# spacejam/loghisto

Hardware: NVIDIA H100
Metric: histogram ingest throughput (samples/s) (higher is better)
Workload: dtype f64

## Files before the change

loghisto_b200/csrc/lh_api.cu:

```cuda
#include "../../include/loghisto_b200.h"
#include "lh_kernels.cuh"

#include <algorithm>
#include <cmath>
#include <condition_variable>
#include <cstdio>
#include <cstring>
#include <mutex>
#include <new>
#include <string>
#include <thread>
#include <vector>
#include <unistd.h>

using namespace lh;

namespace {

struct WriterEvent { cudaStream_t stream; cudaEvent_t ev; };

struct Scope { uint64_t ticket; int buf; cudaStream_t stream; std::thread::id thread; };
static_assert(sizeof(Prec) == sizeof(((lh_recorder *)0)->prec) && offsetof(lh_recorder, prec) % alignof(Prec) == 0,
              "lh_recorder.prec must hold an lh::Prec");

// ... 154 lines not shown
    int nnz_slot = 0;
    short *d_x_keys = nullptr; unsigned long long *d_x_counts = nullptr; size_t x_cap = 0;
    uint32_t *h_offsets = nullptr;
    short *h_x_keys = nullptr; unsigned long long *h_x_counts = nullptr; size_t hx_cap = 0;
    unsigned long long *h_counter_deltas = nullptr;
    std::vector<Slot> slots;
    uint64_t slot_seq = 0;
    size_t staging_bytes = 0;
    unsigned long long last_margin[2] = {0, 0};
    int k1_variant = kDefaultK1Variant;
    int k1_grid_mult = 1;
    int k1_reserve_sms = 0;
    int keyed_blocks_per_sm = 8;
    uint32_t hot_replicas = 1;
    int keyed_mode = 0;
    int64_t kp_chunk = 256 << 20;
    uint32_t wc_pf_tiles = 1;
    uint32_t wc_flush_samples = 24576;
    int wc_spt = 6;
    unsigned short *d_kp_queues = nullptr;
    unsigned int *d_kp_cnt = nullptr;
    uint4 *d_kp_rare = nullptr;
    size_t kp_cap = 0;
    int kp_parts = 0;
    const char *keyed_kernel = "";
    int batch_blocks_per_sm = 1;
    BatchParams batch_prm{};
    uint32_t comm_rank = 0, comm_world = 0;
    unsigned long long *d_comm = nullptr;
    unsigned int *d_comm_aux = nullptr;
    PeerMap peers[kMaxRanks];
    unsigned long long *d_red_buckets = nullptr;
    uint32_t *d_red_flags = nullptr;
    unsigned long long *d_red_counters = nullptr;
// ... 177 lines not shown

template <typename IdT, typename ValT>
void launch_keyed_scalar(lh_ctx *ctx, const KeyedOut &ko, const IdT *ids, const ValT *vals, size_t n, cudaStream_t s,
                         const IdMap *map = nullptr) {
    if (!n) return;
    constexpr int T = 256;
    const int grid = grid_1d(ctx, n, T, 1, ctx->keyed_blocks_per_sm);
    if (map) k_ingest_keyed<IdT, ValT, T, IdMap><<<grid, T, (size_t)map->k * 4, s>>>(ids, vals, n, ko, ctx->pc, *map);
    else k_ingest_keyed<IdT, ValT, T><<<grid, T, 0, s>>>(ids, vals, n, ko, ctx->pc, IdIdentity{});
    ctx->stats.kernel_launches++;
}

constexpr uint32_t KS_MAX_PASSES = 4;

constexpr size_t kSmemBudget = 227 * 1024;

struct KeyedPlan {
    enum Route { SCALAR , SMALL, WC, VEC, APART } route = SCALAR;
    const char *name = "k_ingest_keyed";
    size_t head = 0, n4 = 0;
    size_t taken = 0, taken2 = 0;
    int grid = 0;
    size_t smem = 0;
    uint32_t per = 0;
    int spt = 0, threads = 0;
    WcParams wc{};
};

KeyedPlan plan_keyed(const lh_ctx *ctx, uint32_t nids, size_t id_bytes, const void *ids, const void *vals, size_t n, bool pair = false,
                     const void *ids2 = nullptr, const void *vals2 = nullptr, size_t n2 = 0) {
    KeyedPlan p;
    if (!nids) return p;
    const uint32_t ks_per_max = std::max<uint32_t>(1, (uint32_t)(KS_SMEM_BYTES / ((size_t)ctx->pc.win * 4)));
    const uint32_t ks_passes = (nids + ks_per_max - 1) / ks_per_max;
    const bool small = ks_passes <= KS_MAX_PASSES && ctx->keyed_mode == 0;
    const uintptr_t id_mask = 4 * id_bytes - 1;
    if (pair) {
        auto aligned = [&](const void *v, const void *i) { return ((uintptr_t)v & 31u) == 0 && ((uintptr_t)i & id_mask) == 0; };
        p.route = KeyedPlan::APART;
        if (!n || !n2 || ctx->keyed_mode == 1 || small || !aligned(vals, ids) || !aligned(vals2, ids2)) return p;
// ... 6 lines not shown
        if (small && p.n4 >= 4096) {
            p.route = KeyedPlan::SMALL; p.name = "k_ingest_keyed_small";
            p.per = (nids + ks_passes - 1) / ks_passes;
            p.smem = ((size_t)p.per * ctx->pc.win + 4) * 4;
            p.grid = (int)std::max<size_t>(1, std::min<size_t>((size_t)(ctx->sm_count - ctx->k1_reserve_sms),
                                                               p.n4 / (KS_THREADS * 16)));
            return p;
        }
        p.route = KeyedPlan::VEC; p.name = "k_ingest_keyed_vec";
        if (ctx->keyed_mode == 1) return p;
    }
    const int P = std::min(ctx->sm_count - ctx->k1_reserve_sms, (int)WC_MAX_PARTS);
    if (P < 8) return p;
    const uint32_t ids_per = (nids + P - 1) / P;
    const size_t hist_bytes = (((size_t)ids_per * ctx->pc.win + 3) & ~(size_t)3) * 4;
    uint32_t row_cap = 0;
    size_t smem = 0;
    for (uint32_t cap_try : {256u, 192u, 128u}) {
        smem = hist_bytes + 2 * WC_MAX_PARTS * 4 + (size_t)(P + 1) * (cap_try + WC_ROW_EXTRA) * 2;
        if (smem <= kSmemBudget) { row_cap = cap_try; break; }
    }
    if (!row_cap || (size_t)ids_per * ctx->pc.win > 65535) return p;
    if (ctx->keyed_mode != 2 && n + n2 < ((size_t)1 << 22)) return p;
    const int spt = ctx->wc_spt == 6 || ctx->wc_spt == 4 || ctx->wc_spt == 3 ? ctx->wc_spt : 8;
    const int tile = spt == 6 ? WcShape<6>::TILE : spt == 4 ? WcShape<4>::TILE : spt == 3 ? WcShape<3>::TILE : WcShape<8>::TILE;
    const size_t taken = n / tile * tile, taken2 = n2 / tile * tile;
    if (taken + taken2 == 0) return p;
    p.route = KeyedPlan::WC; p.name = "k_ingest_keyed_wc";
    p.taken = taken; p.taken2 = taken2; p.grid = P; p.smem = smem; p.spt = spt;
    p.threads = spt == 6 ? WcShape<6>::THREADS : spt == 4 ? WcShape<4>::THREADS : spt == 3 ? WcShape<3>::THREADS : WcShape<8>::THREADS;
    WcParams &w = p.wc;
    w.n = taken; w.n2 = taken2; w.ids_per = ids_per; w.row_cap = row_cap; w.row_stride = row_cap + WC_ROW_EXTRA;
    w.inv_p = (uint32_t)(((uint64_t)1 << 32) / (uint64_t)P) + 1u;
    w.pf_tiles = ctx->wc_pf_tiles;
    const size_t slice_max = std::max<size_t>(1, ((size_t)ctx->kp_chunk + (size_t)P * tile - 1) / ((size_t)P * tile));
    const size_t tiles_all = taken / tile + taken2 / tile;
    const size_t nchunks = (tiles_all + slice_max * P - 1) / (slice_max * P);
    w.slice_tiles = (uint32_t)std::max<size_t>(1, (tiles_all + nchunks * P - 1) / (nchunks * P));
    const size_t expect = slice_max * tile / P;
    w.cap = (uint32_t)(((expect * 5 / 4 + 3 * WC_LINE + WC_LINE - 1) / WC_LINE) * WC_LINE);
    const double room = (double)row_cap - 63.0;
    const double m_max = std::pow((-3.5 + std::sqrt(3.5 * 3.5 + 4.0 * room)) / 2.0, 2.0);
    const uint32_t flush_samples = std::min<uint32_t>(ctx->wc_flush_samples, (uint32_t)(m_max * P));
    w.flush_tiles = std::max<uint32_t>(1u, flush_samples / tile);
    return p;
}

std::mutex g_wc_mu;
std::vector<cudaEvent_t> g_wc_done;

cudaError_t wc_done_event(int device, cudaEvent_t *out) {
    if ((size_t)device >= g_wc_done.size()) g_wc_done.resize((size_t)device + 1, nullptr);
    if (!g_wc_done[device]) {
        cudaError_t e = cudaEventCreateWithFlags(&g_wc_done[device], cudaEventDisableTiming);
        if (e != cudaSuccess) { g_wc_done[device] = nullptr; return e; }
    }
    *out = g_wc_done[device];
    return cudaSuccess;
}

template <typename IdT, typename ValT>
lh_status launch_keyed_wc(lh_ctx *ctx, int b, const KeyedPlan &p, const IdT *ids, const ValT *vals, cudaStream_t s,
                          const IdT *ids2 = nullptr, const long long *vals2 = nullptr, const IdMap *map = nullptr) {
    const int P = p.grid;
    if (!ctx->d_kp_queues || ctx->kp_cap != p.wc.cap || ctx->kp_parts != P) {
        if (ctx->d_kp_queues) {
            cudaEvent_t done;
            {
                std::lock_guard<std::mutex> lk(g_wc_mu);
                LH_CUDA(ctx, wc_done_event(ctx->device, &done));
            }
            LH_CUDA(ctx, cudaEventSynchronize(done));
        }
        cudaFree(ctx->d_kp_queues); cudaFree(ctx->d_kp_cnt); cudaFree(ctx->d_kp_rare);
        ctx->d_kp_queues = nullptr; ctx->d_kp_cnt = nullptr; ctx->d_kp_rare = nullptr;
        LH_CUDA(ctx, cudaMalloc(&ctx->d_kp_rare, (size_t)P * WC_RARE_CAP * sizeof(uint4)));
        LH_CUDA(ctx, cudaMalloc(&ctx->d_kp_queues, (size_t)2 * P * P * p.wc.cap * sizeof(unsigned short)));
        LH_CUDA(ctx, cudaMalloc(&ctx->d_kp_cnt, ((size_t)2 * P * P + 1) * sizeof(unsigned int)));
        ctx->kp_cap = p.wc.cap; ctx->kp_parts = P;
    }
#define LH_WC_KERNEL(SPT) (!p.taken2 ? (const void *)k_ingest_keyed_wc<IdT, ValT, SPT, false> : (const void *)k_ingest_keyed_wc<IdT, double, SPT, true>)
    const void *fn = p.spt == 6 ? LH_WC_KERNEL(6) : p.spt == 4 ? LH_WC_KERNEL(4) : p.spt == 3 ? LH_WC_KERNEL(3) : LH_WC_KERNEL(8);
#undef LH_WC_KERNEL
#define LH_WC_MAPPED(SPT) (const void *)k_ingest_keyed_wc<IdT, ValT, SPT, false, IdMap>
    if (map) fn = p.spt == 6 ? LH_WC_MAPPED(6) : p.spt == 4 ? LH_WC_MAPPED(4) : p.spt == 3 ? LH_WC_MAPPED(3) : LH_WC_MAPPED(8);
#undef LH_WC_MAPPED
    LH_CUDA(ctx, cudaFuncSetAttribute(fn, cudaFuncAttributeMaxDynamicSharedMemorySize, (int)kSmemBudget));
    WcParams prm = p.wc;
    prm.ids = ids; prm.vals = vals; prm.ids2 = ids2; prm.vals2 = vals2;
    prm.queues = ctx->d_kp_queues; prm.q_cnt = ctx->d_kp_cnt; prm.barrier = ctx->d_kp_cnt + (size_t)2 * P * P;
    prm.rare = ctx->d_kp_rare; prm.o = keyed_out(ctx, b);
    Prec pc = ctx->pc;
    IdIdentity ident;
    void *args[] = {&prm, &pc, map ? (void *)map : (void *)&ident};
    {
        std::lock_guard<std::mutex> lk(g_wc_mu);
        cudaEvent_t done;
        LH_CUDA(ctx, wc_done_event(ctx->device, &done));
        LH_CUDA(ctx, cudaStreamWaitEvent(s, done, 0));
        LH_CUDA(ctx, cudaMemsetAsync(prm.barrier, 0, sizeof(unsigned int), s));
        LH_CUDA(ctx, cudaLaunchCooperativeKernel(fn, dim3(P), dim3(p.threads), args, p.smem, s));
        LH_CUDA(ctx, cudaEventRecord(done, s));
    }
    ctx->stats.kernel_launches++;
    return LH_OK;
}

template <typename IdT, typename ValT>
lh_status launch_keyed(lh_ctx *ctx, int b, const IdT *d_ids, const ValT *d_vals, size_t n, cudaStream_t s,
                       const IdMap *map = nullptr) {
    constexpr int T = 256;
    const uint32_t nids = map ? map->k : ctx->H;
    const KeyedOut ko = keyed_out(ctx, b);
    size_t done = 0;
    while (done < n) {
        const unsigned long long kCap = 0xFFFFFFFFull;
        if (ctx->buf[b].hot_pending >= kCap - (1ull << 30)) {
            for (const WriterEvent &w : ctx->buf[b].writers)
                if (w.stream != s) LH_CUDA(ctx, cudaStreamWaitEvent(s, w.ev, 0));
// ... 2325 lines not shown
        ctx->keyed_mode = (int)value;
        return LH_OK;
    }
    if (!strcmp(key, "wc_pf")) {
        if (value < 0 || value > 8) return fail(ctx, LH_ERR_RANGE, "wc_pf is 0 ... 8 tiles");
        ctx->wc_pf_tiles = (uint32_t)value;
        return LH_OK;
    }
    if (!strcmp(key, "wc_flush")) {
        if (value < 4096 || value > 65536) return fail(ctx, LH_ERR_RANGE, "wc_flush is 4096 ... 65536 samples");
        ctx->wc_flush_samples = (uint32_t)value;
        return LH_OK;
    }
    if (!strcmp(key, "wc_spt")) {
        if (value != 4 && value != 6 && value != 3 && value != 8)
            return fail(ctx, LH_ERR_RANGE, "wc_spt is a shape code: 6 (896 threads x 4 samples), 4 (1024 x 4), 3 (768 x 4) or 8 (512 x 8)");
        ctx->wc_spt = (int)value;
        return LH_OK;
    }
    if (!strcmp(key, "kp_chunk")) {
        if (value < (1 << 16) || value > ((int64_t)1 << 28)) return fail(ctx, LH_ERR_RANGE, "kp_chunk out of range");
        ctx->kp_chunk = value;
        return LH_OK;
    }
    if (!strcmp(key, "gpu_timer_slots")) {
        if (value < 1 || value > (1 << 20)) return fail(ctx, LH_ERR_RANGE, "gpu_timer_slots is 1 ... 2^20");
        if (ctx->d_timer_marks) return fail(ctx, LH_ERR_STATE, "gpu_timer_slots is set before the first lh_gpu_timer_start");
        ctx->timer_slots_n = (uint32_t)value;
        return LH_OK;
    }
    if (!strcmp(key, "keyed_blocks_per_sm")) {
        if (value < 1 || value > 32) return fail(ctx, LH_ERR_RANGE, "keyed_blocks_per_sm out of range");
        ctx->keyed_blocks_per_sm = (int)value;
        return LH_OK;
    }
    return fail(ctx, LH_ERR_INVALID, "unknown tuning key");
// ... 35 lines not shown
```

loghisto_b200/csrc/lh_kernels.cuh:

```cuda
#pragma once
#include "../../include/loghisto_b200.h"
#include <type_traits>
#include "lh_device.cuh"

namespace lh {

struct f64x4 { double a, b, c, d; };
__device__ __forceinline__ uint64_t policy_evict_first() {
    uint64_t p;
    asm("createpolicy.fractional.L2::evict_first.b64 %0, 1.0;" : "=l"(p));
    return p;
}
__device__ __forceinline__ void ldg_stream_u64x4(const void *p, unsigned long long (&r)[4]) {
    const uint64_t pol = policy_evict_first();
    asm volatile("ld.global.nc.L1::no_allocate.L2::cache_hint.v2.b64 {%0, %1}, [%2], %3;"
                 : "=l"(r[0]), "=l"(r[1]) : "l"(p), "l"(pol));
    asm volatile("ld.global.nc.L1::no_allocate.L2::cache_hint.v2.b64 {%0, %1}, [%2], %3;"
                 : "=l"(r[2]), "=l"(r[3]) : "l"((const char *)p + 16), "l"(pol));
}
__device__ __forceinline__ f64x4 ldg_stream_f64x4(const void *p) {
    unsigned long long u[4];
    ldg_stream_u64x4(p, u);
    f64x4 r;
    r.a = __longlong_as_double((long long)u[0]); r.b = __longlong_as_double((long long)u[1]);
// ... 496 lines not shown
        const uint32_t c = ks_hist[i];
        if (!c) continue;
        const uint32_t lid = i / row, slot = i - lid * row;
        const uint32_t r = mv.row(id_lo + lid);
        if (kMapped<Map> && r == 0xFFFFFFFFu) atomicAdd(o.dropped, (unsigned long long)c);
        else atomicAdd(&o.hot[(size_t)r * (2u * pc.win) + slot], c);
    }
}

constexpr int WC_MAX_PARTS = 160;
constexpr int WC_LINE = 64;

template <int SPT> struct WcShape {
    static constexpr int THREADS = SPT == 4 ? 1024 : SPT == 6 ? 896 : SPT == 3 ? 768 : 512;
    static constexpr int PER = SPT == 8 ? 8 : 4;
    static constexpr int TILE = THREADS * PER;
};
constexpr int WC_ROW_EXTRA = WC_LINE + 8;

struct WcParams {
    const void *ids;
    const void *vals;
    size_t n;
    const void *ids2;
    const void *vals2;
    size_t n2;
    uint32_t ids_per;
    uint32_t cap;
    uint32_t slice_tiles;
    uint32_t inv_p;
    uint32_t flush_tiles;
    uint32_t pf_tiles;
    uint32_t row_cap;
    uint32_t row_stride;
    unsigned short *queues;
    unsigned int *q_cnt;
    unsigned int *barrier;
    uint4 *rare;
    KeyedOut o;
};
constexpr uint32_t WC_RARE_CAP = 8192;

__device__ __forceinline__ void grid_barrier(unsigned int *bar, unsigned int target) {
    __syncthreads();
    if (threadIdx.x == 0) {
        __threadfence();
        atomicAdd(bar, 1u);
        unsigned int v;
        do {
            asm volatile("ld.acquire.gpu.global.u32 %0, [%1];" : "=r"(v) : "l"(bar) : "memory");
        } while (v < target);
    }
    __syncthreads();
}

template <typename V = IdIdentity>
__device__ __forceinline__ void wc_spill(uint32_t rec, uint32_t owner, uint32_t P, const Prec &pc, const KeyedOut &o, const V &m = {}) {
    const uint32_t lid = rec / pc.win, slot = rec - lid * pc.win, id = m.row(lid * P + owner);
    if (kMapped<V> && id == 0xFFFFFFFFu) { atomicAdd(o.dropped, 1ull); return; }
    add_bucket_global(o.buckets + (size_t)id * 65536u, o.flags + id, slot, 1ull, pc.win);
}

template <typename IdT, typename ValT, int SPT, bool PAIR = false, typename Map = IdIdentity>
__global__ void __launch_bounds__(WcShape<SPT>::THREADS, 1)
k_ingest_keyed_wc(WcParams prm, Prec pc, const Map map) {
    static_assert(!PAIR || std::is_same<ValT, double>::value, "the int64 segment rides on the float64 instantiation");
    static_assert(!PAIR || !kMapped<Map>, "pairs are not mapped");
    const auto mv = map_view(map);
    using S = WcShape<SPT>;
    constexpr int WC_THREADS = S::THREADS;
    constexpr int GROUPS = S::PER / 4;
    extern __shared__ __align__(16) unsigned char wc_smem[];
    const uint32_t P = gridDim.x, p = blockIdx.x, tid = threadIdx.x;
    unsigned int *s_hist = reinterpret_cast<unsigned int *>(wc_smem);
    const uint32_t hist_words = prm.ids_per * pc.win;
    unsigned int *s_fill = s_hist + ((hist_words + 3u) & ~3u);
    unsigned int *s_off = s_fill + WC_MAX_PARTS;
    unsigned short *s_buf = reinterpret_cast<unsigned short *>(s_off + WC_MAX_PARTS);
    uint32_t fill_addr = smem_u32(s_fill);
    const uint32_t hist_addr = smem_u32(s_hist);
    asm volatile("mov.b32 %0, %0;" : "+r"(fill_addr));
    const uint32_t buf_addr = fill_addr + 2u * WC_MAX_PARTS * 4u;
    unsigned int *s_rare = s_fill + (WC_MAX_PARTS - 1);
    uint4 *rareq = prm.rare + (size_t)p * WC_RARE_CAP;
    uint32_t negP = 0u - P;
    asm volatile("mov.b32 %0, %0;" : "+r"(negP));

    for (uint32_t i = tid; i < hist_words; i += WC_THREADS) s_hist[i] = 0;
    if (tid < WC_MAX_PARTS) { s_fill[tid] = 0; s_off[tid] = 0; }
    uint32_t one_bits;
    asm volatile("mov.b32 %0, 0x3F800000;" : "=r"(one_bits));
    __syncthreads();

    const size_t tiles_seg0 = prm.n / S::TILE;
    const size_t tiles_total = tiles_seg0 + (PAIR ? prm.n2 / S::TILE : 0);
    const size_t chunk_tiles = (size_t)prm.slice_tiles * P;
    const size_t nchunks = (tiles_total + chunk_tiles - 1) / chunk_tiles;
    const IdT *ids = reinterpret_cast<const IdT *>(prm.ids);
    const unsigned int cap = prm.cap;
    const uint32_t row_cap = prm.row_cap, row_stride = prm.row_stride;


    unsigned long long cur[GROUPS][4], nxt[GROUPS][4];
    IdPack<IdT> cur_id[GROUPS], nxt_id[GROUPS];
    uint32_t since_flush = 0;
    const char *vptr = nullptr;
    const IdT *iptr = nullptr;
    const size_t pf_v = (size_t)prm.pf_tiles * S::TILE * 8, pf_i = (size_t)prm.pf_tiles * S::TILE;
    auto load_tile = [&](const char *vp, const IdT *ip, unsigned long long (&raw)[GROUPS][4], IdPack<IdT> (&idp)[GROUPS]) {
#pragma unroll
        for (int g = 0; g < GROUPS; g++) {
            load_vals4(vp, (size_t)g * WC_THREADS, raw[g]);
            idp[g].load(ip, (size_t)g * WC_THREADS);
        }
    };

    for (size_t c = 0; c < nchunks; c++) {
        const size_t par = c & 1;
        unsigned short *qset = prm.queues + par * (size_t)P * P * cap;
        unsigned int *cset = prm.q_cnt + par * (size_t)P * P;
        const bool last_chunk = c + 1 == nchunks;
        const size_t tile0 = c * chunk_tiles + (size_t)p * prm.slice_tiles;
        const uint32_t ntile_all = tile0 >= tiles_total ? 0u : (uint32_t)min((size_t)prm.slice_tiles, tiles_total - tile0);
        auto bin_tile = [&](unsigned long long (&raw)[GROUPS][4], IdPack<IdT> (&idp)[GROUPS], const bool as_i64) {
            if constexpr (PAIR) {
                if (as_i64) {
#pragma unroll
                    for (int g = 0; g < GROUPS; g++)
#pragma unroll
                        for (int j = 0; j < 4; j++) raw[g][j] = (unsigned long long)__double_as_longlong(__ll2double_rn((long long)raw[g][j]));
                }
            }
#pragma unroll
            for (int g = 0; g < GROUPS; g++) {
                double v[4];
#pragma unroll
                for (int j = 0; j < 4; j++) { ValT r; memcpy(&r, &raw[g][j], 8); v[j] = sample_to_f64<ValT>(r); }
                uint32_t idx[4];
                bool flag[4];
                bucket_offsets_v2<4, false, 0>(v, pc, one_bits, idx, flag);
                bool any = false;
#pragma unroll
                for (int j = 0; j < 4; j++) {
                    const uint32_t id = idp[g].get(j);
                    const uint32_t lid = __umulhi(id, prm.inv_p), owner = lid * negP + id;
                    const uint32_t rec = lid * pc.win + idx[j];
                    const bool rare = flag[j] | (id >= mv.bound(prm.o.H));
                    const uint32_t oe = rare ? P : owner;
                    uint32_t pos;
                    asm volatile("atom.shared.add.u32 %0, [%1], 1;" : "=r"(pos) : "r"(fill_addr + oe * 4u) : "memory");
                    flag[j] = rare | (pos >= row_cap);
                    if (!flag[j])
                        asm volatile("st.shared.u16 [%0], %1;" ::"r"(buf_addr + (oe * row_stride + pos) * 2u), "h"((unsigned short)rec) : "memory");
                    any |= flag[j];
                }
                if (__any_sync(0xFFFFFFFFu, any)) {
#pragma unroll
                    for (int j = 0; j < 4; j++)
                        if (flag[j]) {
                            const unsigned int at = atomicAdd(s_rare, 1u);
                            if (at < WC_RARE_CAP) rareq[at] = make_uint4((unsigned int)raw[g][j], (unsigned int)(raw[g][j] >> 32), idp[g].get(j), 0u);
                            else keyed_one_slow_v<ValT>(idp[g].get(j), raw[g][j], pc, prm.o, mv);
                        }
                }
            }
            if (++since_flush == prm.flush_tiles) {
                since_flush = 0;
                __syncthreads();
                constexpr uint32_t GROUPS_PER_WARP = 8;
                const uint32_t sub = (tid & 31) >> 2, k4 = (tid & 3) * 2;
                for (uint32_t base = (tid >> 5) * GROUPS_PER_WARP; base < P; base += (WC_THREADS / 32) * GROUPS_PER_WARP) {
                    const uint32_t o = base + sub;
                    const bool act = o < P;
                    unsigned int n = 0, nfull = 0, off0 = 0;
                    uint4 keep0 = make_uint4(0, 0, 0, 0), keep1 = keep0;
                    uint4 *src = reinterpret_cast<uint4 *>(s_buf + (act ? o : 0) * row_stride);
                    if (act) {
                        n = min(s_fill[o], row_cap);
                        nfull = n / WC_LINE;
                        off0 = s_off[o];
                        unsigned short *qbase = qset + ((size_t)o * P + p) * cap;
                        keep0 = src[nfull * 8 + k4];
                        keep1 = src[nfull * 8 + k4 + 1];
                        for (unsigned int l = 0; l < nfull; l++) {
                            if (off0 + WC_LINE <= cap) {
                                uint4 *dst = reinterpret_cast<uint4 *>(qbase + off0);
                                const uint4 a0 = src[l * 8 + k4], a1 = src[l * 8 + k4 + 1];
                                dst[k4] = a0;
                                dst[k4 + 1] = a1;
                                off0 += WC_LINE;
                            } else if (k4 == 0) {
                                const unsigned short *r = s_buf + o * row_stride + l * WC_LINE;
                                for (unsigned int k = 0; k < (unsigned int)WC_LINE; k++) wc_spill(r[k], o, P, pc, prm.o, mv);
                            }
                        }
                    }
                    __syncwarp();
                    if (act) {
                        if (nfull) { src[k4] = keep0; src[k4 + 1] = keep1; }
                        if (k4 == 0) { s_off[o] = off0; s_fill[o] = n - nfull * WC_LINE; }
                    }
                }
                __syncthreads();
            }
        };
        for (int part = 0; part < (PAIR ? 2 : 1); part++) {
            const size_t lo = part == 0 ? tile0 : max(tile0, tiles_seg0);
            const size_t hi = part == 0 ? min(tile0 + ntile_all, tiles_seg0) : tile0 + ntile_all;
            if (hi <= lo) continue;
            const uint32_t ntile = (uint32_t)(hi - lo);
            const bool as_i64 = part == 1;
            const size_t first = (part == 0 ? lo : lo - tiles_seg0) * S::TILE + (size_t)tid * 4;
            vptr = reinterpret_cast<const char *>(part == 0 ? prm.vals : prm.vals2) + first * 8;
            iptr = (part == 0 ? ids : reinterpret_cast<const IdT *>(prm.ids2)) + first;
            load_tile(vptr, iptr, cur, cur_id);
            auto prefetch_ahead = [&](uint32_t tile_loaded) {
                if (prm.pf_tiles && tile_loaded + prm.pf_tiles < ntile) {
#pragma unroll
                    for (int g = 0; g < GROUPS; g++) {
                        asm volatile("prefetch.global.L2 [%0];" ::"l"(vptr + pf_v + (size_t)g * WC_THREADS * 32));
                        if ((tid & 3) == 0) asm volatile("prefetch.global.L2 [%0];" ::"l"(iptr + pf_i + (size_t)g * WC_THREADS * 4));
                    }
                }
            };
            for (uint32_t t = 0; t < ntile; t += 2) {
                vptr += (size_t)S::TILE * 8;
                iptr += S::TILE;
                if (t + 1 < ntile) load_tile(vptr, iptr, nxt, nxt_id);
                prefetch_ahead(t + 1);
                bin_tile(cur, cur_id, as_i64);
                if (t + 1 >= ntile) break;
                vptr += (size_t)S::TILE * 8;
                iptr += S::TILE;
                if (t + 2 < ntile) load_tile(vptr, iptr, cur, cur_id);
                prefetch_ahead(t + 2);
                bin_tile(nxt, nxt_id, as_i64);
            }
        }
        __syncthreads();
        {
            const unsigned int nr = min(*s_rare, WC_RARE_CAP);
            for (unsigned int i = tid; i < nr; i += WC_THREADS) {
                const uint4 e = rareq[i];
                ValT r;
                const unsigned long long raw = ((unsigned long long)e.y << 32) | e.x;
                memcpy(&r, &raw, 8);
                keyed_one_direct<ValT>(e.z, r, pc, prm.o, mv);
            }
            __syncthreads();
            if (tid == 0) *s_rare = 0;
        }
        if (last_chunk) {
            if (tid < P) {
                const uint32_t o = tid;
                const unsigned int n = min(s_fill[o], row_cap);
                unsigned int off0 = s_off[o];
                const uint4 *src = reinterpret_cast<const uint4 *>(s_buf + o * row_stride);
                for (unsigned int l = 0; l * WC_LINE < n; l++) {
                    const unsigned int nrec = min((unsigned int)WC_LINE, n - l * WC_LINE);
                    if (off0 + WC_LINE <= cap) {
                        uint4 *dst = reinterpret_cast<uint4 *>(qset + ((size_t)o * P + p) * cap + off0);
#pragma unroll
                        for (int k = 0; k < 8; k++) dst[k] = src[l * 8 + k];
                        off0 += nrec;
                    } else {
                        const unsigned short *r = s_buf + o * row_stride + l * WC_LINE;
                        for (unsigned int k = 0; k < nrec; k++) wc_spill(r[k], o, P, pc, prm.o, mv);
                    }
                }
                s_off[o] = off0;
                s_fill[o] = 0;
            }
            __syncthreads();
        }
        if (tid < P) { cset[(size_t)tid * P + p] = s_off[tid]; }
        grid_barrier(prm.barrier, (unsigned int)((c + 1) * (size_t)P));
        if (tid < P) s_off[tid] = __ldcg(&cset[(size_t)p * P + tid]);
        __syncthreads();
        {
            const unsigned short *qmine = qset + (size_t)p * P * cap;
            const uint32_t lane = tid & 31;
#define LH_WC_INC2(word)                                                                                              \
            asm volatile("red.shared.add.u32 [%0], 1;" ::"r"(hist_addr + (((word) << 2) & 0x3FFFCu)) : "memory");     \
            asm volatile("red.shared.add.u32 [%0], 1;" ::"r"(hist_addr + (((word) >> 14) & 0x3FFFCu)) : "memory");
            for (uint32_t w = tid >> 5; w < P; w += WC_THREADS / 32) {
                const unsigned int cnt = s_off[w];
                const unsigned short *q = qmine + (size_t)w * cap;
                const uint4 *qv = reinterpret_cast<const uint4 *>(q);
                const unsigned int nv = cnt >> 3;
#pragma unroll 2
                for (unsigned int i = lane; i < nv; i += 32) {
                    const uint4 v4 = __ldcg(qv + i);
                    LH_WC_INC2(v4.x) LH_WC_INC2(v4.y) LH_WC_INC2(v4.z) LH_WC_INC2(v4.w)
                }
                const unsigned int r0 = nv * 8u + lane;
                if (r0 < cnt) asm volatile("red.shared.add.u32 [%0], 1;" ::"r"(hist_addr + (unsigned int)__ldcg(q + r0) * 4u) : "memory");
            }
#undef LH_WC_INC2
        }
        __syncthreads();
        if (tid < P) s_off[tid] = 0;
    }
    __syncthreads();
    for (uint32_t lid = 0; lid < prm.ids_per; lid++) {
        if (lid * P + p >= mv.bound(prm.o.H)) break;
        const uint32_t id = mv.row(lid * P + p);
        if (kMapped<Map> && id == 0xFFFFFFFFu) {
            unsigned long long lost = 0;
            for (uint32_t slot = tid; slot < pc.win; slot += WC_THREADS) lost += s_hist[lid * pc.win + slot];
            if (lost) atomicAdd(prm.o.dropped, lost);
            continue;
        }
        int any = 0;
        for (uint32_t slot = tid; slot < pc.win; slot += WC_THREADS) {
            const unsigned int cnt = s_hist[lid * pc.win + slot];
            if (cnt) { atomicAdd(&prm.o.buckets[(size_t)id * 65536u + slot], (unsigned long long)cnt); any = 1; }
        }
        any = __syncthreads_or(any);
        if (any && tid == 0) mark(&prm.o.flags[id], 1u);
    }
}

__global__ void k_fold_hot(unsigned int *__restrict__ hot, unsigned long long *__restrict__ buckets, uint32_t *__restrict__ flags,
                           size_t cells, uint32_t replicas, uint32_t win) {
    const size_t stride = (size_t)gridDim.x * blockDim.x;
    const uint32_t row = 2u * win;
    for (size_t i = (size_t)blockIdx.x * blockDim.x + threadIdx.x; i < cells; i += stride) {
        unsigned long long sum = 0;
        for (uint32_t r = 0; r < replicas; r++) {
// ... 1587 lines not shown
```

Measured before the change: 399.4 billion.

## Split cooperative keyed write-combine kernel into per-chunk bin and drain launches

Replaces the single cooperative kernel, which used software grid barriers and double-buffered queues, with two ordinary kernels per chunk. The first bins samples using twice as many writer CTAs, two per SM, each with a smaller shared budget. The second drains the queues into per-owner shared histograms. This removes the grid-barrier spin and the large per-CTA shared footprint in exchange for extra launches, re-zeroing and flushing the histograms on every chunk, and losing overlap between binning and draining. Defaults also change to a larger chunk and the 3-sample shape.

```diff
diff --git a/loghisto_b200/csrc/lh_api.cu b/loghisto_b200/csrc/lh_api.cu
--- a/loghisto_b200/csrc/lh_api.cu
+++ b/loghisto_b200/csrc/lh_api.cu
@@ -192,10 +192,10 @@
     int keyed_blocks_per_sm = 8;
     uint32_t hot_replicas = 1;
     int keyed_mode = 0;
-    int64_t kp_chunk = 256 << 20;
+    int64_t kp_chunk = 512 << 20;
     uint32_t wc_pf_tiles = 1;
     uint32_t wc_flush_samples = 24576;
-    int wc_spt = 6;
+    int wc_spt = 3;
     unsigned short *d_kp_queues = nullptr;
     unsigned int *d_kp_cnt = nullptr;
     uint4 *d_kp_rare = nullptr;
@@ -403,6 +403,8 @@
 constexpr uint32_t KS_MAX_PASSES = 4;
 
 constexpr size_t kSmemBudget = 227 * 1024;
+constexpr size_t kBinSmemBudget = 113 * 1024;
+constexpr size_t kWcQueueBytes = (size_t)5 << 28;
 
 struct KeyedPlan {
     enum Route { SCALAR , SMALL, WC, VEC, APART } route = SCALAR;
@@ -413,6 +415,8 @@
     size_t smem = 0;
     uint32_t per = 0;
     int spt = 0, threads = 0;
+    size_t drain_smem = 0;
+    uint32_t nchunks = 0;
     WcParams wc{};
 };
 
@@ -449,29 +453,31 @@
     if (P < 8) return p;
     const uint32_t ids_per = (nids + P - 1) / P;
     const size_t hist_bytes = (((size_t)ids_per * ctx->pc.win + 3) & ~(size_t)3) * 4;
-    uint32_t row_cap = 0;
-    size_t smem = 0;
-    for (uint32_t cap_try : {256u, 192u, 128u}) {
-        smem = hist_bytes + 2 * WC_MAX_PARTS * 4 + (size_t)(P + 1) * (cap_try + WC_ROW_EXTRA) * 2;
-        if (smem <= kSmemBudget) { row_cap = cap_try; break; }
-    }
-    if (!row_cap || (size_t)ids_per * ctx->pc.win > 65535) return p;
+    bool reach = false;
+    for (uint32_t cap_try : {256u, 192u, 128u})
+        reach = reach || hist_bytes + 2 * WC_MAX_PARTS * 4 + (size_t)(P + 1) * (cap_try + WC_ROW_EXTRA) * 2 <= kSmemBudget;
+    if (!reach || (size_t)ids_per * ctx->pc.win > 65535) return p;
     if (ctx->keyed_mode != 2 && n + n2 < ((size_t)1 << 22)) return p;
-    const int spt = ctx->wc_spt == 6 || ctx->wc_spt == 4 || ctx->wc_spt == 3 ? ctx->wc_spt : 8;
-    const int tile = spt == 6 ? WcShape<6>::TILE : spt == 4 ? WcShape<4>::TILE : spt == 3 ? WcShape<3>::TILE : WcShape<8>::TILE;
+    const int spt = ctx->wc_spt == 8 ? 8 : 3;
+    const int tile = spt == 3 ? WcShape<3>::TILE : WcShape<8>::TILE;
     const size_t taken = n / tile * tile, taken2 = n2 / tile * tile;
     if (taken + taken2 == 0) return p;
+    const int W = 2 * P;
+    const uint32_t row_cap = (uint32_t)(((kBinSmemBudget - wc_bin_smem(P, 0)) / ((size_t)(P + 1) * 2) - WC_ROW_EXTRA) / WC_LINE * WC_LINE);
     p.route = KeyedPlan::WC; p.name = "k_ingest_keyed_wc";
-    p.taken = taken; p.taken2 = taken2; p.grid = P; p.smem = smem; p.spt = spt;
-    p.threads = spt == 6 ? WcShape<6>::THREADS : spt == 4 ? WcShape<4>::THREADS : spt == 3 ? WcShape<3>::THREADS : WcShape<8>::THREADS;
+    p.taken = taken; p.taken2 = taken2; p.grid = P; p.spt = spt;
+    p.threads = spt == 3 ? WcShape<3>::CTA_THREADS : WcShape<8>::CTA_THREADS;
+    p.smem = wc_bin_smem(P, row_cap + WC_ROW_EXTRA);
+    p.drain_smem = hist_bytes + (size_t)W * 4;
     WcParams &w = p.wc;
-    w.n = taken; w.n2 = taken2; w.ids_per = ids_per; w.row_cap = row_cap; w.row_stride = row_cap + WC_ROW_EXTRA;
+    w.n = taken; w.n2 = taken2; w.parts = P; w.writers = W; w.ids_per = ids_per; w.row_cap = row_cap; w.row_stride = row_cap + WC_ROW_EXTRA;
     w.inv_p = (uint32_t)(((uint64_t)1 << 32) / (uint64_t)P) + 1u;
     w.pf_tiles = ctx->wc_pf_tiles;
-    const size_t slice_max = std::max<size_t>(1, ((size_t)ctx->kp_chunk + (size_t)P * tile - 1) / ((size_t)P * tile));
+    const size_t chunk = std::min<size_t>((size_t)ctx->kp_chunk, kWcQueueBytes * 2 / 5);
+    const size_t slice_max = std::max<size_t>(1, (chunk + (size_t)W * tile - 1) / ((size_t)W * tile));
     const size_t tiles_all = taken / tile + taken2 / tile;
-    const size_t nchunks = (tiles_all + slice_max * P - 1) / (slice_max * P);
-    w.slice_tiles = (uint32_t)std::max<size_t>(1, (tiles_all + nchunks * P - 1) / (nchunks * P));
+    p.nchunks = (uint32_t)((tiles_all + slice_max * W - 1) / (slice_max * W));
+    w.slice_tiles = (uint32_t)std::max<size_t>(1, (tiles_all + (size_t)p.nchunks * W - 1) / ((size_t)p.nchunks * W));
     const size_t expect = slice_max * tile / P;
     w.cap = (uint32_t)(((expect * 5 / 4 + 3 * WC_LINE + WC_LINE - 1) / WC_LINE) * WC_LINE);
     const double room = (double)row_cap - 63.0;
@@ -497,7 +503,7 @@
 template <typename IdT, typename ValT>
 lh_status launch_keyed_wc(lh_ctx *ctx, int b, const KeyedPlan &p, const IdT *ids, const ValT *vals, cudaStream_t s,
                           const IdT *ids2 = nullptr, const long long *vals2 = nullptr, const IdMap *map = nullptr) {
-    const int P = p.grid;
+    const int P = p.grid, W = (int)p.wc.writers;
     if (!ctx->d_kp_queues || ctx->kp_cap != p.wc.cap || ctx->kp_parts != P) {
         if (ctx->d_kp_queues) {
             cudaEvent_t done;
@@ -509,21 +515,21 @@
         }
         cudaFree(ctx->d_kp_queues); cudaFree(ctx->d_kp_cnt); cudaFree(ctx->d_kp_rare);
         ctx->d_kp_queues = nullptr; ctx->d_kp_cnt = nullptr; ctx->d_kp_rare = nullptr;
-        LH_CUDA(ctx, cudaMalloc(&ctx->d_kp_rare, (size_t)P * WC_RARE_CAP * sizeof(uint4)));
-        LH_CUDA(ctx, cudaMalloc(&ctx->d_kp_queues, (size_t)2 * P * P * p.wc.cap * sizeof(unsigned short)));
-        LH_CUDA(ctx, cudaMalloc(&ctx->d_kp_cnt, ((size_t)2 * P * P + 1) * sizeof(unsigned int)));
+        LH_CUDA(ctx, cudaMalloc(&ctx->d_kp_rare, (size_t)W * WC_RARE_CAP * sizeof(uint4)));
+        LH_CUDA(ctx, cudaMalloc(&ctx->d_kp_queues, (size_t)P * W * p.wc.cap * sizeof(unsigned short)));
+        LH_CUDA(ctx, cudaMalloc(&ctx->d_kp_cnt, (size_t)P * W * sizeof(unsigned int)));
         ctx->kp_cap = p.wc.cap; ctx->kp_parts = P;
     }
-#define LH_WC_KERNEL(SPT) (!p.taken2 ? (const void *)k_ingest_keyed_wc<IdT, ValT, SPT, false> : (const void *)k_ingest_keyed_wc<IdT, double, SPT, true>)
-    const void *fn = p.spt == 6 ? LH_WC_KERNEL(6) : p.spt == 4 ? LH_WC_KERNEL(4) : p.spt == 3 ? LH_WC_KERNEL(3) : LH_WC_KERNEL(8);
+#define LH_WC_KERNEL(SPT) (map ? (const void *)k_keyed_bin<IdT, ValT, SPT, false, IdMap> : !p.taken2 ? (const void *)k_keyed_bin<IdT, ValT, SPT, false> \
+                                                                                    : (const void *)k_keyed_bin<IdT, double, SPT, true>)
+    const void *bin = p.spt == 3 ? LH_WC_KERNEL(3) : LH_WC_KERNEL(8);
 #undef LH_WC_KERNEL
-#define LH_WC_MAPPED(SPT) (const void *)k_ingest_keyed_wc<IdT, ValT, SPT, false, IdMap>
-    if (map) fn = p.spt == 6 ? LH_WC_MAPPED(6) : p.spt == 4 ? LH_WC_MAPPED(4) : p.spt == 3 ? LH_WC_MAPPED(3) : LH_WC_MAPPED(8);
-#undef LH_WC_MAPPED
-    LH_CUDA(ctx, cudaFuncSetAttribute(fn, cudaFuncAttributeMaxDynamicSharedMemorySize, (int)kSmemBudget));
+    const void *drain = map ? (const void *)k_keyed_drain<IdMap> : (const void *)k_keyed_drain<IdIdentity>;
+    LH_CUDA(ctx, cudaFuncSetAttribute(bin, cudaFuncAttributeMaxDynamicSharedMemorySize, (int)kBinSmemBudget));
+    LH_CUDA(ctx, cudaFuncSetAttribute(drain, cudaFuncAttributeMaxDynamicSharedMemorySize, (int)kSmemBudget));
     WcParams prm = p.wc;
     prm.ids = ids; prm.vals = vals; prm.ids2 = ids2; prm.vals2 = vals2;
-    prm.queues = ctx->d_kp_queues; prm.q_cnt = ctx->d_kp_cnt; prm.barrier = ctx->d_kp_cnt + (size_t)2 * P * P;
+    prm.queues = ctx->d_kp_queues; prm.q_cnt = ctx->d_kp_cnt;
     prm.rare = ctx->d_kp_rare; prm.o = keyed_out(ctx, b);
     Prec pc = ctx->pc;
     IdIdentity ident;
@@ -533,11 +539,14 @@
         cudaEvent_t done;
         LH_CUDA(ctx, wc_done_event(ctx->device, &done));
         LH_CUDA(ctx, cudaStreamWaitEvent(s, done, 0));
-        LH_CUDA(ctx, cudaMemsetAsync(prm.barrier, 0, sizeof(unsigned int), s));
-        LH_CUDA(ctx, cudaLaunchCooperativeKernel(fn, dim3(P), dim3(p.threads), args, p.smem, s));
+        for (uint32_t c = 0; c < p.nchunks; c++) {
+            prm.tile0 = (size_t)c * p.wc.slice_tiles * W;
+            LH_CUDA(ctx, cudaLaunchKernel(bin, dim3(W), dim3(p.threads), args, p.smem, s));
+            LH_CUDA(ctx, cudaLaunchKernel(drain, dim3(P), dim3(KD_THREADS), args, p.drain_smem, s));
+        }
         LH_CUDA(ctx, cudaEventRecord(done, s));
     }
-    ctx->stats.kernel_launches++;
+    ctx->stats.kernel_launches += 2 * (uint64_t)p.nchunks;
     return LH_OK;
 }
 
@@ -2893,12 +2902,12 @@
     }
     if (!strcmp(key, "wc_spt")) {
         if (value != 4 && value != 6 && value != 3 && value != 8)
-            return fail(ctx, LH_ERR_RANGE, "wc_spt is a shape code: 6 (896 threads x 4 samples), 4 (1024 x 4), 3 (768 x 4) or 8 (512 x 8)");
+            return fail(ctx, LH_ERR_RANGE, "wc_spt is a shape code: 3 (768 threads per SM x 4 samples) or 8 (512 x 8); 6 and 4 run as 3");
         ctx->wc_spt = (int)value;
         return LH_OK;
     }
     if (!strcmp(key, "kp_chunk")) {
-        if (value < (1 << 16) || value > ((int64_t)1 << 28)) return fail(ctx, LH_ERR_RANGE, "kp_chunk out of range");
+        if (value < (1 << 16) || value > ((int64_t)1 << 30)) return fail(ctx, LH_ERR_RANGE, "kp_chunk out of range");
         ctx->kp_chunk = value;
         return LH_OK;
     }
diff --git a/loghisto_b200/csrc/lh_kernels.cuh b/loghisto_b200/csrc/lh_kernels.cuh
--- a/loghisto_b200/csrc/lh_kernels.cuh
+++ b/loghisto_b200/csrc/lh_kernels.cuh
@@ -534,9 +534,11 @@
 template <int SPT> struct WcShape {
     static constexpr int THREADS = SPT == 4 ? 1024 : SPT == 6 ? 896 : SPT == 3 ? 768 : 512;
     static constexpr int PER = SPT == 8 ? 8 : 4;
-    static constexpr int TILE = THREADS * PER;
+    static constexpr int CTA_THREADS = THREADS / 2;
+    static constexpr int TILE = CTA_THREADS * PER;
 };
 constexpr int WC_ROW_EXTRA = WC_LINE + 8;
+constexpr int KD_THREADS = 1024;
 
 struct WcParams {
     const void *ids;
@@ -545,6 +547,9 @@
     const void *ids2;
     const void *vals2;
     size_t n2;
+    size_t tile0;
+    uint32_t parts;
+    uint32_t writers;
     uint32_t ids_per;
     uint32_t cap;
     uint32_t slice_tiles;
@@ -555,23 +560,14 @@
     uint32_t row_stride;
     unsigned short *queues;
     unsigned int *q_cnt;
-    unsigned int *barrier;
     uint4 *rare;
     KeyedOut o;
 };
 constexpr uint32_t WC_RARE_CAP = 8192;
 
-__device__ __forceinline__ void grid_barrier(unsigned int *bar, unsigned int target) {
-    __syncthreads();
-    if (threadIdx.x == 0) {
-        __threadfence();
-        atomicAdd(bar, 1u);
-        unsigned int v;
-        do {
-            asm volatile("ld.acquire.gpu.global.u32 %0, [%1];" : "=r"(v) : "l"(bar) : "memory");
-        } while (v < target);
-    }
-    __syncthreads();
+constexpr uint32_t WC_BIN_HEAD = 2 * WC_MAX_PARTS + 4;
+__host__ __device__ constexpr size_t wc_bin_smem(uint32_t P, uint32_t row_stride) {
+    return (size_t)WC_BIN_HEAD * 4 + (size_t)(P + 1) * row_stride * 2;
 }
 
 template <typename V = IdIdentity>
@@ -582,44 +578,38 @@
 }
 
 template <typename IdT, typename ValT, int SPT, bool PAIR = false, typename Map = IdIdentity>
-__global__ void __launch_bounds__(WcShape<SPT>::THREADS, 1)
-k_ingest_keyed_wc(WcParams prm, Prec pc, const Map map) {
+__global__ void __launch_bounds__(WcShape<SPT>::CTA_THREADS, 2)
+k_keyed_bin(WcParams prm, Prec pc, const Map map) {
     static_assert(!PAIR || std::is_same<ValT, double>::value, "the int64 segment rides on the float64 instantiation");
     static_assert(!PAIR || !kMapped<Map>, "pairs are not mapped");
     const auto mv = map_view(map);
     using S = WcShape<SPT>;
-    constexpr int WC_THREADS = S::THREADS;
+    constexpr int WC_THREADS = S::CTA_THREADS;
     constexpr int GROUPS = S::PER / 4;
     extern __shared__ __align__(16) unsigned char wc_smem[];
-    const uint32_t P = gridDim.x, p = blockIdx.x, tid = threadIdx.x;
-    unsigned int *s_hist = reinterpret_cast<unsigned int *>(wc_smem);
-    const uint32_t hist_words = prm.ids_per * pc.win;
-    unsigned int *s_fill = s_hist + ((hist_words + 3u) & ~3u);
-    unsigned int *s_off = s_fill + WC_MAX_PARTS;
-    unsigned short *s_buf = reinterpret_cast<unsigned short *>(s_off + WC_MAX_PARTS);
+    const uint32_t P = prm.parts, W = prm.writers, w = blockIdx.x, tid = threadIdx.x;
+    unsigned int *s_fill = reinterpret_cast<unsigned int *>(wc_smem);
+    unsigned int *s_rare = s_fill + WC_MAX_PARTS + 1;
+    unsigned int *s_off = s_fill + WC_MAX_PARTS + 2;
+    unsigned short *s_buf = reinterpret_cast<unsigned short *>(s_fill + WC_BIN_HEAD);
     uint32_t fill_addr = smem_u32(s_fill);
-    const uint32_t hist_addr = smem_u32(s_hist);
     asm volatile("mov.b32 %0, %0;" : "+r"(fill_addr));
-    const uint32_t buf_addr = fill_addr + 2u * WC_MAX_PARTS * 4u;
-    unsigned int *s_rare = s_fill + (WC_MAX_PARTS - 1);
-    uint4 *rareq = prm.rare + (size_t)p * WC_RARE_CAP;
+    const uint32_t buf_addr = fill_addr + WC_BIN_HEAD * 4u;
+    uint4 *rareq = prm.rare + (size_t)w * WC_RARE_CAP;
     uint32_t negP = 0u - P;
     asm volatile("mov.b32 %0, %0;" : "+r"(negP));
-
-    for (uint32_t i = tid; i < hist_words; i += WC_THREADS) s_hist[i] = 0;
-    if (tid < WC_MAX_PARTS) { s_fill[tid] = 0; s_off[tid] = 0; }
+    unsigned short *qset = prm.queues;
+
+    for (uint32_t i = tid; i < WC_BIN_HEAD; i += WC_THREADS) s_fill[i] = 0;
     uint32_t one_bits;
     asm volatile("mov.b32 %0, 0x3F800000;" : "=r"(one_bits));
     __syncthreads();
 
     const size_t tiles_seg0 = prm.n / S::TILE;
     const size_t tiles_total = tiles_seg0 + (PAIR ? prm.n2 / S::TILE : 0);
-    const size_t chunk_tiles = (size_t)prm.slice_tiles * P;
-    const size_t nchunks = (tiles_total + chunk_tiles - 1) / chunk_tiles;
     const IdT *ids = reinterpret_cast<const IdT *>(prm.ids);
     const unsigned int cap = prm.cap;
     const uint32_t row_cap = prm.row_cap, row_stride = prm.row_stride;
-
 
     unsigned long long cur[GROUPS][4], nxt[GROUPS][4];
     IdPack<IdT> cur_id[GROUPS], nxt_id[GROUPS];
@@ -635,191 +625,187 @@
         }
     };
 
-    for (size_t c = 0; c < nchunks; c++) {
-        const size_t par = c & 1;
-        unsigned short *qset = prm.queues + par * (size_t)P * P * cap;
-        unsigned int *cset = prm.q_cnt + par * (size_t)P * P;
-        const bool last_chunk = c + 1 == nchunks;
-        const size_t tile0 = c * chunk_tiles + (size_t)p * prm.slice_tiles;
-        const uint32_t ntile_all = tile0 >= tiles_total ? 0u : (uint32_t)min((size_t)prm.slice_tiles, tiles_total - tile0);
-        auto bin_tile = [&](unsigned long long (&raw)[GROUPS][4], IdPack<IdT> (&idp)[GROUPS], const bool as_i64) {
-            if constexpr (PAIR) {
-                if (as_i64) {
-#pragma unroll
-                    for (int g = 0; g < GROUPS; g++)
-#pragma unroll
-                        for (int j = 0; j < 4; j++) raw[g][j] = (unsigned long long)__double_as_longlong(__ll2double_rn((long long)raw[g][j]));
-                }
-            }
-#pragma unroll
-            for (int g = 0; g < GROUPS; g++) {
-                double v[4];
-#pragma unroll
-                for (int j = 0; j < 4; j++) { ValT r; memcpy(&r, &raw[g][j], 8); v[j] = sample_to_f64<ValT>(r); }
-                uint32_t idx[4];
-                bool flag[4];
-                bucket_offsets_v2<4, false, 0>(v, pc, one_bits, idx, flag);
-                bool any = false;
-#pragma unroll
-                for (int j = 0; j < 4; j++) {
-                    const uint32_t id = idp[g].get(j);
-                    const uint32_t lid = __umulhi(id, prm.inv_p), owner = lid * negP + id;
-                    const uint32_t rec = lid * pc.win + idx[j];
-                    const bool rare = flag[j] | (id >= mv.bound(prm.o.H));
-                    const uint32_t oe = rare ? P : owner;
-                    uint32_t pos;
-                    asm volatile("atom.shared.add.u32 %0, [%1], 1;" : "=r"(pos) : "r"(fill_addr + oe * 4u) : "memory");
-                    flag[j] = rare | (pos >= row_cap);
-                    if (!flag[j])
-                        asm volatile("st.shared.u16 [%0], %1;" ::"r"(buf_addr + (oe * row_stride + pos) * 2u), "h"((unsigned short)rec) : "memory");
-                    any |= flag[j];
-                }
-                if (__any_sync(0xFFFFFFFFu, any)) {
-#pragma unroll
-                    for (int j = 0; j < 4; j++)
-                        if (flag[j]) {
-                            const unsigned int at = atomicAdd(s_rare, 1u);
-                            if (at < WC_RARE_CAP) rareq[at] = make_uint4((unsigned int)raw[g][j], (unsigned int)(raw[g][j] >> 32), idp[g].get(j), 0u);
-                            else keyed_one_slow_v<ValT>(idp[g].get(j), raw[g][j], pc, prm.o, mv);
-                        }
-                }
-            }
-            if (++since_flush == prm.flush_tiles) {
-                since_flush = 0;
-                __syncthreads();
-                constexpr uint32_t GROUPS_PER_WARP = 8;
-                const uint32_t sub = (tid & 31) >> 2, k4 = (tid & 3) * 2;
-                for (uint32_t base = (tid >> 5) * GROUPS_PER_WARP; base < P; base += (WC_THREADS / 32) * GROUPS_PER_WARP) {
-                    const uint32_t o = base + sub;
-                    const bool act = o < P;
-                    unsigned int n = 0, nfull = 0, off0 = 0;
-                    uint4 keep0 = make_uint4(0, 0, 0, 0), keep1 = keep0;
-                    uint4 *src = reinterpret_cast<uint4 *>(s_buf + (act ? o : 0) * row_stride);
-                    if (act) {
-                        n = min(s_fill[o], row_cap);
-                        nfull = n / WC_LINE;
-                        off0 = s_off[o];
-                        unsigned short *qbase = qset + ((size_t)o * P + p) * cap;
-                        keep0 = src[nfull * 8 + k4];
-                        keep1 = src[nfull * 8 + k4 + 1];
-                        for (unsigned int l = 0; l < nfull; l++) {
-                            if (off0 + WC_LINE <= cap) {
-                                uint4 *dst = reinterpret_cast<uint4 *>(qbase + off0);
-                                const uint4 a0 = src[l * 8 + k4], a1 = src[l * 8 + k4 + 1];
-                                dst[k4] = a0;
-                                dst[k4 + 1] = a1;
-                                off0 += WC_LINE;
-                            } else if (k4 == 0) {
-                                const unsigned short *r = s_buf + o * row_stride + l * WC_LINE;
-                                for (unsigned int k = 0; k < (unsigned int)WC_LINE; k++) wc_spill(r[k], o, P, pc, prm.o, mv);
-                            }
+    const size_t tile0 = prm.tile0 + (size_t)w * prm.slice_tiles;
+    const uint32_t ntile_all = tile0 >= tiles_total ? 0u : (uint32_t)min((size_t)prm.slice_tiles, tiles_total - tile0);
+    auto bin_tile = [&](unsigned long long (&raw)[GROUPS][4], IdPack<IdT> (&idp)[GROUPS], const bool as_i64) {
+        if constexpr (PAIR) {
+            if (as_i64) {
+#pragma unroll
+                for (int g = 0; g < GROUPS; g++)
+#pragma unroll
+                    for (int j = 0; j < 4; j++) raw[g][j] = (unsigned long long)__double_as_longlong(__ll2double_rn((long long)raw[g][j]));
+            }
+        }
+#pragma unroll
+        for (int g = 0; g < GROUPS; g++) {
+            double v[4];
+#pragma unroll
+            for (int j = 0; j < 4; j++) { ValT r; memcpy(&r, &raw[g][j], 8); v[j] = sample_to_f64<ValT>(r); }
+            uint32_t idx[4];
+            bool flag[4];
+            bucket_offsets_v2<4, false, 0>(v, pc, one_bits, idx, flag);
+            bool any = false;
+#pragma unroll
+            for (int j = 0; j < 4; j++) {
+                const uint32_t id = idp[g].get(j);
+                const uint32_t lid = __umulhi(id, prm.inv_p), owner = lid * negP + id;
+                const uint32_t rec = lid * pc.win + idx[j];
+                const bool rare = flag[j] | (id >= mv.bound(prm.o.H));
+                const uint32_t oe = rare ? P : owner;
+                uint32_t pos;
+                asm volatile("atom.shared.add.u32 %0, [%1], 1;" : "=r"(pos) : "r"(fill_addr + oe * 4u) : "memory");
+                flag[j] = rare | (pos >= row_cap);
+                if (!flag[j])
+                    asm volatile("st.shared.u16 [%0], %1;" ::"r"(buf_addr + (oe * row_stride + pos) * 2u), "h"((unsigned short)rec) : "memory");
+                any |= flag[j];
+            }
+            if (__any_sync(0xFFFFFFFFu, any)) {
+#pragma unroll
+                for (int j = 0; j < 4; j++)
+                    if (flag[j]) {
+                        const unsigned int at = atomicAdd(s_rare, 1u);
+                        if (at < WC_RARE_CAP) rareq[at] = make_uint4((unsigned int)raw[g][j], (unsigned int)(raw[g][j] >> 32), idp[g].get(j), 0u);
+                        else keyed_one_slow_v<ValT>(idp[g].get(j), raw[g][j], pc, prm.o, mv);
+                    }
+            }
+        }
+        if (++since_flush == prm.flush_tiles) {
+            since_flush = 0;
+            __syncthreads();
+            constexpr uint32_t GROUPS_PER_WARP = 8;
+            const uint32_t sub = (tid & 31) >> 2, k4 = (tid & 3) * 2;
+            for (uint32_t base = (tid >> 5) * GROUPS_PER_WARP; base < P; base += (WC_THREADS / 32) * GROUPS_PER_WARP) {
+                const uint32_t o = base + sub;
+                const bool act = o < P;
+                unsigned int n = 0, nfull = 0, off0 = 0;
+                uint4 keep0 = make_uint4(0, 0, 0, 0), keep1 = keep0;
+                uint4 *src = reinterpret_cast<uint4 *>(s_buf + (act ? o : 0) * row_stride);
+                if (act) {
+                    n = min(s_fill[o], row_cap);
+                    nfull = n / WC_LINE;
+                    off0 = s_off[o];
+                    unsigned short *qbase = qset + ((size_t)o * W + w) * cap;
+                    keep0 = src[nfull * 8 + k4];
+                    keep1 = src[nfull * 8 + k4 + 1];
+                    for (unsigned int l = 0; l < nfull; l++) {
+                        if (off0 + WC_LINE <= cap) {
+                            uint4 *dst = reinterpret_cast<uint4 *>(qbase + off0);
+                            const uint4 a0 = src[l * 8 + k4], a1 = src[l * 8 + k4 + 1];
+                            dst[k4] = a0;
+                            dst[k4 + 1] = a1;
+                            off0 += WC_LINE;
+                        } else if (k4 == 0) {
+                            const unsigned short *r = s_buf + o * row_stride + l * WC_LINE;
+                            for (unsigned int k = 0; k < (unsigned int)WC_LINE; k++) wc_spill(r[k], o, P, pc, prm.o, mv);
                         }
                     }
-                    __syncwarp();
-                    if (act) {
-                        if (nfull) { src[k4] = keep0; src[k4 + 1] = keep1; }
-                        if (k4 == 0) { s_off[o] = off0; s_fill[o] = n - nfull * WC_LINE; }
-                    }
                 }
-                __syncthreads();
+                __syncwarp();
+                if (act) {
+                    if (nfull) { src[k4] = keep0; src[k4 + 1] = keep1; }
+                    if (k4 == 0) { s_off[o] = off0; s_fill[o] = n - nfull * WC_LINE; }
+                }
+            }
+            __syncthreads();
+        }
+    };
+    for (int part = 0; part < (PAIR ? 2 : 1); part++) {
+        const size_t lo = part == 0 ? tile0 : max(tile0, tiles_seg0);
+        const size_t hi = part == 0 ? min(tile0 + ntile_all, tiles_seg0) : tile0 + ntile_all;
+        if (hi <= lo) continue;
+        const uint32_t ntile = (uint32_t)(hi - lo);
+        const bool as_i64 = part == 1;
+        const size_t first = (part == 0 ? lo : lo - tiles_seg0) * S::TILE + (size_t)tid * 4;
+        vptr = reinterpret_cast<const char *>(part == 0 ? prm.vals : prm.vals2) + first * 8;
+        iptr = (part == 0 ? ids : reinterpret_cast<const IdT *>(prm.ids2)) + first;
+        load_tile(vptr, iptr, cur, cur_id);
+        auto prefetch_ahead = [&](uint32_t tile_loaded) {
+            if (prm.pf_tiles && tile_loaded + prm.pf_tiles < ntile) {
+#pragma unroll
+                for (int g = 0; g < GROUPS; g++) {
+                    asm volatile("prefetch.global.L2 [%0];" ::"l"(vptr + pf_v + (size_t)g * WC_THREADS * 32));
+                    if ((tid & 3) == 0) asm volatile("prefetch.global.L2 [%0];" ::"l"(iptr + pf_i + (size_t)g * WC_THREADS * 4));
+                }
             }
         };
-        for (int part = 0; part < (PAIR ? 2 : 1); part++) {
-            const size_t lo = part == 0 ? tile0 : max(tile0, tiles_seg0);
-            const size_t hi = part == 0 ? min(tile0 + ntile_all, tiles_seg0) : tile0 + ntile_all;
-            if (hi <= lo) continue;
-            const uint32_t ntile = (uint32_t)(hi - lo);
-            const bool as_i64 = part == 1;
-            const size_t first = (part == 0 ? lo : lo - tiles_seg0) * S::TILE + (size_t)tid * 4;
-            vptr = reinterpret_cast<const char *>(part == 0 ? prm.vals : prm.vals2) + first * 8;
-            iptr = (part == 0 ? ids : reinterpret_cast<const IdT *>(prm.ids2)) + first;
-            load_tile(vptr, iptr, cur, cur_id);
-            auto prefetch_ahead = [&](uint32_t tile_loaded) {
-                if (prm.pf_tiles && tile_loaded + prm.pf_tiles < ntile) {
-#pragma unroll
-                    for (int g = 0; g < GROUPS; g++) {
-                        asm volatile("prefetch.global.L2 [%0];" ::"l"(vptr + pf_v + (size_t)g * WC_THREADS * 32));
-                        if ((tid & 3) == 0) asm volatile("prefetch.global.L2 [%0];" ::"l"(iptr + pf_i + (size_t)g * WC_THREADS * 4));
-                    }
-                }
-            };
-            for (uint32_t t = 0; t < ntile; t += 2) {
-                vptr += (size_t)S::TILE * 8;
-                iptr += S::TILE;
-                if (t + 1 < ntile) load_tile(vptr, iptr, nxt, nxt_id);
-                prefetch_ahead(t + 1);
-                bin_tile(cur, cur_id, as_i64);
-                if (t + 1 >= ntile) break;
-                vptr += (size_t)S::TILE * 8;
-                iptr += S::TILE;
-                if (t + 2 < ntile) load_tile(vptr, iptr, cur, cur_id);
-                prefetch_ahead(t + 2);
-                bin_tile(nxt, nxt_id, as_i64);
-            }
-        }
-        __syncthreads();
-        {
-            const unsigned int nr = min(*s_rare, WC_RARE_CAP);
-            for (unsigned int i = tid; i < nr; i += WC_THREADS) {
-                const uint4 e = rareq[i];
-                ValT r;
-                const unsigned long long raw = ((unsigned long long)e.y << 32) | e.x;
-                memcpy(&r, &raw, 8);
-                keyed_one_direct<ValT>(e.z, r, pc, prm.o, mv);
-            }
-            __syncthreads();
-            if (tid == 0) *s_rare = 0;
-        }
-        if (last_chunk) {
-            if (tid < P) {
-                const uint32_t o = tid;
-                const unsigned int n = min(s_fill[o], row_cap);
-                unsigned int off0 = s_off[o];
-                const uint4 *src = reinterpret_cast<const uint4 *>(s_buf + o * row_stride);
-                for (unsigned int l = 0; l * WC_LINE < n; l++) {
-                    const unsigned int nrec = min((unsigned int)WC_LINE, n - l * WC_LINE);
-                    if (off0 + WC_LINE <= cap) {
-                        uint4 *dst = reinterpret_cast<uint4 *>(qset + ((size_t)o * P + p) * cap + off0);
-#pragma unroll
-                        for (int k = 0; k < 8; k++) dst[k] = src[l * 8 + k];
-                        off0 += nrec;
-                    } else {
-                        const unsigned short *r = s_buf + o * row_stride + l * WC_LINE;
-                        for (unsigned int k = 0; k < nrec; k++) wc_spill(r[k], o, P, pc, prm.o, mv);
-                    }
-                }
-                s_off[o] = off0;
-                s_fill[o] = 0;
-            }
-            __syncthreads();
-        }
-        if (tid < P) { cset[(size_t)tid * P + p] = s_off[tid]; }
-        grid_barrier(prm.barrier, (unsigned int)((c + 1) * (size_t)P));
-        if (tid < P) s_off[tid] = __ldcg(&cset[(size_t)p * P + tid]);
-        __syncthreads();
-        {
-            const unsigned short *qmine = qset + (size_t)p * P * cap;
-            const uint32_t lane = tid & 31;
+        for (uint32_t t = 0; t < ntile; t += 2) {
+            vptr += (size_t)S::TILE * 8;
+            iptr += S::TILE;
+            if (t + 1 < ntile) load_tile(vptr, iptr, nxt, nxt_id);
+            prefetch_ahead(t + 1);
+            bin_tile(cur, cur_id, as_i64);
+            if (t + 1 >= ntile) break;
+            vptr += (size_t)S::TILE * 8;
+            iptr += S::TILE;
+            if (t + 2 < ntile) load_tile(vptr, iptr, cur, cur_id);
+            prefetch_ahead(t + 2);
+            bin_tile(nxt, nxt_id, as_i64);
+        }
+    }
+    __syncthreads();
+    {
+        const unsigned int nr = min(*s_rare, WC_RARE_CAP);
+        for (unsigned int i = tid; i < nr; i += WC_THREADS) {
+            const uint4 e = rareq[i];
+            ValT r;
+            const unsigned long long raw = ((unsigned long long)e.y << 32) | e.x;
+            memcpy(&r, &raw, 8);
+            keyed_one_direct<ValT>(e.z, r, pc, prm.o, mv);
+        }
+    }
+    for (uint32_t o = tid; o < P; o += WC_THREADS) {
+        const unsigned int n = min(s_fill[o], row_cap);
+        unsigned int off0 = s_off[o];
+        const uint4 *src = reinterpret_cast<const uint4 *>(s_buf + o * row_stride);
+        for (unsigned int l = 0; l * WC_LINE < n; l++) {
+            const unsigned int nrec = min((unsigned int)WC_LINE, n - l * WC_LINE);
+            if (off0 + WC_LINE <= cap) {
+                uint4 *dst = reinterpret_cast<uint4 *>(qset + ((size_t)o * W + w) * cap + off0);
+#pragma unroll
+                for (int k = 0; k < 8; k++) dst[k] = src[l * 8 + k];
+                off0 += nrec;
+            } else {
+                const unsigned short *r = s_buf + o * row_stride + l * WC_LINE;
+                for (unsigned int k = 0; k < nrec; k++) wc_spill(r[k], o, P, pc, prm.o, mv);
+            }
+        }
+        prm.q_cnt[(size_t)o * W + w] = off0;
+    }
+}
+
+template <typename Map = IdIdentity>
+__global__ void __launch_bounds__(KD_THREADS, 1)
+k_keyed_drain(WcParams prm, Prec pc, const Map map) {
+    const auto mv = map_view(map);
+    extern __shared__ __align__(16) unsigned char wc_smem[];
+    const uint32_t P = gridDim.x, W = prm.writers, p = blockIdx.x, tid = threadIdx.x;
+    unsigned int *s_hist = reinterpret_cast<unsigned int *>(wc_smem);
+    const uint32_t hist_words = prm.ids_per * pc.win;
+    unsigned int *s_cnt = s_hist + ((hist_words + 3u) & ~3u);
+    const uint32_t hist_addr = smem_u32(s_hist);
+    for (uint32_t i = tid; i < hist_words; i += KD_THREADS) s_hist[i] = 0;
+    for (uint32_t i = tid; i < W; i += KD_THREADS) s_cnt[i] = __ldcg(&prm.q_cnt[(size_t)p * W + i]);
+    __syncthreads();
+    {
+        const unsigned short *qmine = prm.queues + (size_t)p * W * prm.cap;
+        const uint32_t lane = tid & 31;
 #define LH_WC_INC2(word)                                                                                              \
-            asm volatile("red.shared.add.u32 [%0], 1;" ::"r"(hist_addr + (((word) << 2) & 0x3FFFCu)) : "memory");     \
-            asm volatile("red.shared.add.u32 [%0], 1;" ::"r"(hist_addr + (((word) >> 14) & 0x3FFFCu)) : "memory");
-            for (uint32_t w = tid >> 5; w < P; w += WC_THREADS / 32) {
-                const unsigned int cnt = s_off[w];
-                const unsigned short *q = qmine + (size_t)w * cap;
-                const uint4 *qv = reinterpret_cast<const uint4 *>(q);
-                const unsigned int nv = cnt >> 3;
+        asm volatile("red.shared.add.u32 [%0], 1;" ::"r"(hist_addr + (((word) << 2) & 0x3FFFCu)) : "memory");     \
+        asm volatile("red.shared.add.u32 [%0], 1;" ::"r"(hist_addr + (((word) >> 14) & 0x3FFFCu)) : "memory");
+        for (uint32_t v = tid >> 5; v < W; v += KD_THREADS / 32) {
+            const unsigned int cnt = s_cnt[v];
+            const unsigned short *q = qmine + (size_t)v * prm.cap;
+            const uint4 *qv = reinterpret_cast<const uint4 *>(q);
+            const unsigned int nv = cnt >> 3;
 #pragma unroll 2
-                for (unsigned int i = lane; i < nv; i += 32) {
-                    const uint4 v4 = __ldcg(qv + i);
-                    LH_WC_INC2(v4.x) LH_WC_INC2(v4.y) LH_WC_INC2(v4.z) LH_WC_INC2(v4.w)
-                }
-                const unsigned int r0 = nv * 8u + lane;
-                if (r0 < cnt) asm volatile("red.shared.add.u32 [%0], 1;" ::"r"(hist_addr + (unsigned int)__ldcg(q + r0) * 4u) : "memory");
-            }
+            for (unsigned int i = lane; i < nv; i += 32) {
+                const uint4 v4 = __ldcg(qv + i);
+                LH_WC_INC2(v4.x) LH_WC_INC2(v4.y) LH_WC_INC2(v4.z) LH_WC_INC2(v4.w)
+            }
+            const unsigned int r0 = nv * 8u + lane;
+            if (r0 < cnt) asm volatile("red.shared.add.u32 [%0], 1;" ::"r"(hist_addr + (unsigned int)__ldcg(q + r0) * 4u) : "memory");
+        }
 #undef LH_WC_INC2
-        }
-        __syncthreads();
-        if (tid < P) s_off[tid] = 0;
     }
     __syncthreads();
     for (uint32_t lid = 0; lid < prm.ids_per; lid++) {
@@ -827,12 +813,12 @@
         const uint32_t id = mv.row(lid * P + p);
         if (kMapped<Map> && id == 0xFFFFFFFFu) {
             unsigned long long lost = 0;
-            for (uint32_t slot = tid; slot < pc.win; slot += WC_THREADS) lost += s_hist[lid * pc.win + slot];
+            for (uint32_t slot = tid; slot < pc.win; slot += KD_THREADS) lost += s_hist[lid * pc.win + slot];
             if (lost) atomicAdd(prm.o.dropped, lost);
             continue;
         }
         int any = 0;
-        for (uint32_t slot = tid; slot < pc.win; slot += WC_THREADS) {
+        for (uint32_t slot = tid; slot < pc.win; slot += KD_THREADS) {
             const unsigned int cnt = s_hist[lid * pc.win + slot];
             if (cnt) { atomicAdd(&prm.o.buckets[(size_t)id * 65536u + slot], (unsigned long long)cnt); any = 1; }
         }
```

Measured after the change: 399.3 billion, median of 6. Within noise of the previous version (-0.0%).
